# epfl-lts2/pygsp

Measured on AMD Instinct MI355X. Metric: filtered-vertices/sec (N·Nsig·K/s) + achieved HBM GB/s vs roofline, 1M-vertex K=30, higher is better.
Workload: dtype f64

## Files before the change

pygsp_amd/csrc/gspx_ctx.hip.h:

```cpp
#pragma once

struct Options {
  int64_t kernel = 0;
  int64_t vec = 0;
  int64_t rows_per_wave = 0;
  int64_t narrow_g_log2 = -1;
  int64_t waves_per_block = 4;
  int64_t calib_mix = 0;
  int64_t graph_launch = 2;
  int64_t tile_gather = 1;
  int64_t tile_workgroups = 0;
  int64_t knn_f32 = 1;
  int64_t tile_pad = 1;
  int64_t tile_min_row = 16;
  int64_t staged_copy = 1;
  int64_t staged_copy_min_mb = 32;
  int64_t copy_threads = 0;
  int64_t tile_regroup = 1;
  int64_t tile_acc_builds = 1;
  int64_t tile_lg = 0;
  int64_t edge_vertex_walk = 1;
  int64_t fuse_input = 1;
  int64_t tile_nt = -1;
  int64_t synthesis = 0;
  int64_t alternate_sweep = 1;
  int64_t xcd_remap = 1;
  int64_t combine = 0;
  int64_t ws_limit_mb = 65536;
  int64_t max_batch = 0;
  int64_t gather_rccl = 1;
  int64_t lds_pad_kb = 0;
  int64_t host_pipeline = 1;
  int64_t host_batch = 0;
  int64_t host_edge = 0;
  int64_t host_threads = 0;
  int64_t streamed_alloc = 1;
  int64_t layout_splits = 0;
};

struct gspx_ctx {
  int device = 0;
  int cu_count = 256;
  hipStream_t stream = nullptr;
  Options opt;
  DevMem ws_t;
  DevMem ws_r;
  DevMem ws_w;
  DevMem io_x, io_y;
  DevMem ws_spec;
  DevMem ws_sq, ws_sqp;
  HostPipe* pipe = nullptr;
  CopyStage* copy = nullptr;
  bool counted = false;
  std::mutex comms_mu;
  std::vector<struct gspx_comm*> comms;
  hipEvent_t ev[4] = {nullptr, nullptr, nullptr, nullptr};
  std::vector<hipEvent_t> ev_pool;
  double timing[5] = {0, 0, 0, 0, 0};
  int64_t step_kinds[2] = {0, 0};
  bool capturing = false;
  std::vector<unsigned char> seen_key;
  std::vector<unsigned char> graph_key;
  hipGraphExec_t graph_exec = nullptr;
  int64_t graph_kinds[2] = {0, 0};
};

static std::atomic<int> g_live_ctx[64];

static void replay_reset(gspx_ctx* ctx) {
  if (!ctx) return;
  ctx->seen_key.clear();
  ctx->graph_key.clear();
  if (ctx->graph_exec) {
    (void)hipGraphExecDestroy(ctx->graph_exec);
    ctx->graph_exec = nullptr;
  }
}

static int finish_timed(gspx_ctx* ctx, double* kernel_ms) {
  HIPCHK(hipGetLastError());
  HIPCHK(hipStreamSynchronize(ctx->stream));
  float f = 0;
  HIPCHK(hipEventElapsedTime(&f, ctx->ev[0], ctx->ev[1]));
  if (kernel_ms) *kernel_ms = f;
  return GSPX_OK;
}

struct gspx_buf {
  gspx_ctx* ctx = nullptr;
  DevMem mem;
  int64_t bytes = 0;
};

static std::atomic<uint64_t> g_generation{1};

struct gspx_graph {
  gspx_ctx* ctx = nullptr;
  const uint64_t generation = g_generation.fetch_add(1);
  int64_t N = 0;
  int dtype = GSPX_F64;
  bool from_w = false;
  int64_t nnz_l = 0;
// ... 93 lines not shown
    return set_err(GSPX_ERR_HIP, "hipStreamCreate failed: %s", hipGetErrorString(e));
  }
  for (int i = 0; i < 4; ++i) {
    e = hipEventCreate(&ctx->ev[i]);
    if (e != hipSuccess) {
      delete ctx;
      return set_err(GSPX_ERR_HIP, "hipEventCreate failed: %s", hipGetErrorString(e));
    }
  }
  *out = ctx;
  return GSPX_OK;
}

static void comm_invalidate_all(gspx_ctx* ctx);

extern "C" int gspx_ctx_destroy(gspx_ctx* ctx) {
  replay_reset(ctx);
  if (!ctx) return GSPX_OK;
  if (ctx->counted) g_live_ctx[ctx->device & 63].fetch_sub(1);
  comm_invalidate_all(ctx);
  if (ctx->graph_exec) {
    (void)hipGraphExecDestroy(ctx->graph_exec);
    ctx->graph_exec = nullptr;
  }
  (void)hipSetDevice(ctx->device);
  if (ctx->stream) (void)hipStreamSynchronize(ctx->stream);
  for (int i = 0; i < 4; ++i)
    if (ctx->ev[i]) (void)hipEventDestroy(ctx->ev[i]);
  for (hipEvent_t e : ctx->ev_pool) (void)hipEventDestroy(e);
  ctx->ws_t.release();
  ctx->ws_r.release();
  ctx->ws_w.release();
  ctx->io_x.release();
  ctx->io_y.release();
  ctx->ws_spec.release();
  ctx->ws_sq.release();
  ctx->ws_sqp.release();
  if (ctx->pipe) {
    ctx->pipe->destroy();
    delete ctx->pipe;
    ctx->pipe = nullptr;
  }
  if (ctx->copy) {
    ctx->copy->destroy();
    delete ctx->copy;
    ctx->copy = nullptr;
  }
  if (ctx->stream) (void)hipStreamDestroy(ctx->stream);
  delete ctx;
  return GSPX_OK;
}

extern "C" int gspx_ctx_sync(gspx_ctx* ctx) {
  if (!ctx) return set_err(GSPX_ERR_INVALID, "null ctx");
  HIPCHK(hipSetDevice(ctx->device));
  HIPCHK(hipStreamSynchronize(ctx->stream));
  return GSPX_OK;
}

struct OptionDef {
  const char* key;
  int64_t Options::*slot;
  bool (*ok)(int64_t);
  const char* refusal;
};
static const OptionDef OPTION_TABLE[] = {
    {"kernel", &Options::kernel, [](int64_t v) { return v == 0 || v == 1 || v == 2 || v == 5; },
     "kernel must be 0 (auto), 1 (panel), 2 (narrow) or 5 (LDS-staged)"},
    {"vec", &Options::vec, [](int64_t v) { return v == 0 || v == 1 || v == 2 || v == 4; }, "vec must be 0, 1, 2 or 4"},
    {"rows_per_wave", &Options::rows_per_wave, [](int64_t v) { return v >= 0 && v <= 1024; },
     "rows_per_wave must be in [0, 1024] (0 = auto)"},
    {"narrow_g_log2", &Options::narrow_g_log2, [](int64_t v) { return v >= -1 && v <= 6; },
     "narrow_g_log2 must be in [-1, 6] (-1 = auto)"},
    {"waves_per_block", &Options::waves_per_block, [](int64_t v) { return v == 4 || v == 8 || v == 16; },
     "waves_per_block must be 4, 8 or 16"},
    {"alternate_sweep", &Options::alternate_sweep, nullptr, nullptr},
    {"synthesis", &Options::synthesis, nullptr, nullptr},
    {"tile_gather", &Options::tile_gather, nullptr, nullptr},
    {"graph_launch", &Options::graph_launch, nullptr, nullptr},
    {"tile_workgroups", &Options::tile_workgroups, nullptr, nullptr},
    {"tile_lg", &Options::tile_lg, nullptr, nullptr},
    {"tile_regroup", &Options::tile_regroup, nullptr, nullptr},
    {"tile_acc_builds", &Options::tile_acc_builds, nullptr, nullptr},
    {"staged_copy", &Options::staged_copy, nullptr, nullptr},
    {"staged_copy_min_mb", &Options::staged_copy_min_mb, nullptr, nullptr},
    {"copy_threads", &Options::copy_threads, nullptr, nullptr},
    {"tile_min_row", &Options::tile_min_row, nullptr, nullptr},
    {"tile_pad", &Options::tile_pad, nullptr, nullptr},
    {"knn_f32", &Options::knn_f32, nullptr, nullptr},
    {"tile_nt", &Options::tile_nt, nullptr, nullptr},
    {"fuse_input", &Options::fuse_input, nullptr, nullptr},
    {"edge_vertex_walk", &Options::edge_vertex_walk, nullptr, nullptr},
    {"xcd_remap", &Options::xcd_remap, nullptr, nullptr},
    {"combine", &Options::combine, nullptr, nullptr},
    {"ws_limit_mb", &Options::ws_limit_mb, nullptr, nullptr},
    {"max_batch", &Options::max_batch, nullptr, nullptr},
    {"gather_rccl", &Options::gather_rccl, nullptr, nullptr},
    {"lds_pad_kb", &Options::lds_pad_kb, nullptr, nullptr},
    {"host_pipeline", &Options::host_pipeline, nullptr, nullptr},
    {"host_batch", &Options::host_batch, nullptr, nullptr},
    {"host_edge", &Options::host_edge, nullptr, nullptr},
    {"host_threads", &Options::host_threads, nullptr, nullptr},
    {"streamed_alloc", &Options::streamed_alloc, nullptr, nullptr},
    {"layout_splits", &Options::layout_splits, [](int64_t v) { return v >= 0 && v <= 65535; },
     "layout_splits must be in [0, 65535] (0 = automatic)"},
};

static const OptionDef* find_option(const char* key) {
  if (key)
    for (const OptionDef& d : OPTION_TABLE)
      if (!strcmp(key, d.key)) return &d;
  set_err(GSPX_ERR_INVALID, "unknown option '%s'", key ? key : "(null)");
  return nullptr;
}

extern "C" int gspx_ctx_set_option(gspx_ctx* ctx, const char* key, int64_t value) {
  replay_reset(ctx);
  if (!ctx) return set_err(GSPX_ERR_INVALID, "null ctx");
  const OptionDef* d = find_option(key);
  if (!d) return GSPX_ERR_INVALID;
  if (d->ok && !d->ok(value)) return set_err(GSPX_ERR_INVALID, "%s", d->refusal);
  ctx->opt.*d->slot = value;
  if (d->slot == &Options::streamed_alloc) {
    const bool on = value != 0;
    (void)hipSetDevice(ctx->device);
    for (DevMem* m : {&ctx->ws_t, &ctx->ws_r}) {
      if (!on && m->va_size) {
        (void)hipStreamSynchronize(ctx->stream);
        m->release();
      }
      m->streamed = on;
    }
  }
  return GSPX_OK;
}

extern "C" int gspx_ctx_get_option(gspx_ctx* ctx, const char* key, int64_t* value) {
  if (!ctx || !value) return set_err(GSPX_ERR_INVALID, "null argument");
  if (key && !strcmp(key, "retired_va_mb")) {
    *value = (int64_t)(g_retired_va_bytes.load() >> 20);
    return GSPX_OK;
  }
  const OptionDef* d = find_option(key);
  if (!d) return GSPX_ERR_INVALID;
  *value = ctx->opt.*d->slot;
  return GSPX_OK;
}

extern "C" int gspx_buf_alloc(gspx_ctx* ctx, int64_t bytes, gspx_buf** out) {
  if (!ctx || !out || bytes < 0) return set_err(GSPX_ERR_INVALID, "gspx_buf_alloc: bad argument");
  *out = nullptr;
  HIPCHK(hipSetDevice(ctx->device));
  gspx_buf* b = new gspx_buf();
  b->ctx = ctx;
  b->bytes = bytes;
  int rc = b->mem.alloc((size_t)bytes);
  if (rc != GSPX_OK) {
    delete b;
    return rc;
  }
  *out = b;
  return GSPX_OK;
}

extern "C" int gspx_buf_free(gspx_buf* b) {
  if (!b) return GSPX_OK;
// ... 170 lines not shown
```

pygsp_amd/csrc/gspx_poly.hip.h:

```cpp
#pragma once

struct PlanStep {
  double scale = 1.0, gamma = -1.0;
  int flush = 0;
  int final = 0;
  std::vector<double> w;
};

static void make_plan_fused(int nf, int M, const std::vector<double>& cp, bool acc_existing,
                            bool final_to_y, std::vector<PlanStep>& plan) {
  const int K = M - 1;
  plan.assign((size_t)K, PlanStep());
  int covered = -1;
  bool first = !acc_existing;
  for (int k = 1; k <= K; ++k) {
    PlanStep& st = plan[(size_t)k - 1];
    st.scale = (k == 1) ? 0.5 : 1.0;
    st.gamma = (k == 1) ? 0.0 : -1.0;
    st.w.assign((size_t)nf * 3, 0.0);
    const bool must = (k == K) || (k >= 2 && (k - 2) > covered);
    if (!must) continue;
    st.flush = first ? 1 : 2;
    first = false;
    st.final = (k == K && final_to_y) ? 1 : 0;
// ... 311 lines not shown
  if constexpr (sizeof(T) == 4) {
    if (vec == 2) kern = k_slot_dots<T, 2, 8>;
  }
  hipLaunchKernelGGL(kern, grid, dim3(256), 0, st, slots, S, slot_stride, (u32)pitch, N, (int)w, cwl, sd.part);
  const int64_t n = (int64_t)(2 * S - 1) * w;
  hipLaunchKernelGGL(k_dots_reduce, dim3((unsigned)((n + 63) / 64)), dim3(256), 0, st, sd.part, gx, n, (int)w, sd.out,
                     sd.ldo);
  return GSPX_OK;
}

struct CrossDots {
  const void* z;
  unsigned ldz;
  size_t zplane;
  int nf;
  double* out;
  size_t ldo;
  double* part;
};
static const int CROSS_PASS = 8, CROSS_FEW = 2;
static int cross_cs(int here, int vec) { return (here <= CROSS_FEW ? 16 : 8) / vec; }
template <typename T> static int cross_vec(unsigned w, unsigned pitch, const T* z, unsigned ldz) {
  return dots_vec<T>(w, pitch) == 2 && ldz % 2 == 0 && ((uintptr_t)z % (2 * sizeof(T))) == 0 ? 2 : 1;
}
static int cross_chunks(int M, int here, int vec) { return (M + cross_cs(here, vec) - 1) / cross_cs(here, vec); }
static int cross_gx(const gspx_ctx* ctx, int N, unsigned w, int M, int here, int vec) {
  const int cwl = sqnorm_cwl(w / vec);
  const int64_t rows = 4 * (int64_t)(64 >> cwl);
  const int64_t tiles = ((int64_t)N + rows - 1) / rows;
  const int64_t others = (((int64_t)(w / vec) + (1 << cwl) - 1) >> cwl) * cross_chunks(M, here, vec);
  const int64_t fit = ((int64_t)64 << 20) / ((int64_t)here * M * w * (int64_t)sizeof(double));
  const int64_t want = (8 * (int64_t)ctx->cu_count + others - 1) / others;
  return (int)std::max<int64_t>(1, std::min(std::min(tiles, want), fit));
}
static size_t cross_parts(const gspx_ctx* ctx, int N, unsigned w, int M, int nf) {
  size_t most = 0;
  for (int here : {std::min(nf, CROSS_PASS), nf % CROSS_PASS})
    for (int vec = 1; here > 0 && vec <= (w % 2 == 0 ? 2 : 1); ++vec)
      most = std::max(most, (size_t)cross_gx(ctx, N, w, M, here, vec) * (size_t)here * M * w);
  return most;
}

template <typename T>
static int launch_slot_cross_dots(gspx_ctx* ctx, const T* slots, int M, size_t slot_stride, unsigned pitch, int N,
                                  unsigned w, const int* perm, const CrossDots& cd, hipStream_t st) {
  const T* z = (const T*)cd.z;
  const int vec = cross_vec<T>(w, pitch, z, cd.ldz);
  const int cwl = sqnorm_cwl(w / vec);
  typedef void (*kern_t)(const T*, int, size_t, u32, const T*, int, size_t, u32, const int*, int, int, int, double*);
  for (int f0 = 0; f0 < cd.nf; f0 += CROSS_PASS) {
    const int here = std::min(CROSS_PASS, cd.nf - f0);
    const bool few = here <= CROSS_FEW;
    kern_t kern = few ? k_slot_cross_dots<T, 1, 16, CROSS_FEW> : k_slot_cross_dots<T, 1, 8, CROSS_PASS>;
    if constexpr (sizeof(T) == 4) {
      if (vec == 2) kern = few ? k_slot_cross_dots<T, 2, 8, CROSS_FEW> : k_slot_cross_dots<T, 2, 4, CROSS_PASS>;
    }
    const int gx = cross_gx(ctx, N, w, M, here, vec);
    const dim3 grid((unsigned)gx, (unsigned)cross_chunks(M, here, vec), (w / vec + (1u << cwl) - 1) >> cwl);
    hipLaunchKernelGGL(kern, grid, dim3(256), 0, st, slots, M, slot_stride, (u32)pitch, z + (size_t)f0 * cd.zplane, here,
                       cd.zplane, (u32)cd.ldz, perm, N, (int)w, cwl, cd.part);
    const int64_t n = (int64_t)here * M * w;
    hipLaunchKernelGGL(k_dots_reduce, dim3((unsigned)((n + 63) / 64)), dim3(256), 0, st, cd.part, gx, n, (int)w,
                       cd.out + (size_t)f0 * M * cd.ldo, cd.ldo);
  }
  return GSPX_OK;
}

struct SlotsUse {
  int (*fn)(gspx_ctx*, const void*, int, size_t, unsigned, int, unsigned, const int*, const void*, hipStream_t);
  const void* arg;
};

template <typename T> static bool tile_geometry(const gspx_graph* g, const Options& opt, unsigned ld) {
  constexpr int TVEC = 16 / (int)sizeof(T);
  const size_t U = (size_t)g->N * ld;
  return opt.tile_gather && g->gt_rows == GSPX_TILE_BR && (size_t)ld * sizeof(T) >= (size_t)opt.tile_min_row &&
         (ld % TVEC) == 0 && U * sizeof(T) < ((size_t)1 << 31) && (size_t)g->nnz_int * sizeof(T) < ((size_t)1 << 31);
}
template <typename T>
static bool tile_usable(const gspx_graph* g, const Options& opt, unsigned ld, const T* y, unsigned ldy) {
  constexpr int TVEC = 16 / (int)sizeof(T);
  return tile_geometry<T>(g, opt, ld) && (ldy % TVEC) == 0 && (((uintptr_t)y / sizeof(T)) % TVEC) == 0;
}
template <typename T>
static int launch_step_tile(gspx_graph* g, const Options& opt, TileArgs<T> t, unsigned ld, hipStream_t st,
                            const T* vals = nullptr) {
  const size_t rowb = (size_t)ld * sizeof(T);
  int lg = rowb <= 16 ? 1 : rowb <= 32 ? 2 : rowb <= 64 ? 4 : rowb <= 128 ? 8 : 16;
  if (opt.tile_lg == 8 || opt.tile_lg == 4 || opt.tile_lg == 2) lg = rowb <= 128 ? std::max(lg, (int)opt.tile_lg) : 16;
  const bool narrow = lg < 16;
  const int ncol = narrow ? 1 : (int)((rowb + 255) / 256);
  const int flavour = t.old_rows ? 1 : t.nin > 0 ? 2 : 0;
  typedef void (*kern_t)(const TileArgs<T>);
  static const kern_t wide[3][3] = {
      {k_step_tile<T, 0>, k_step_tile<T, 1>, k_step_tile<T, 2>},
      {k_step_tile<T, 0, 16, true>, k_step_tile<T, 1, 16, true>, k_step_tile<T, 2, 16, true>},
      {k_step_tile<T, 0, 16, false, true>, k_step_tile<T, 1, 16, false, true>, k_step_tile<T, 2, 16, false, true>}};
  static const kern_t slim[3][4] = {
      {k_step_tile<T, 1, 1, false, false, 64>, k_step_tile<T, 1, 2, false, false, 128>,
       k_step_tile<T, 1, 4, false, false, 256>, k_step_tile<T, 1, 8>},
      {k_step_tile<T, 1, 1, true, false, 64>, k_step_tile<T, 1, 2, true, false, 128>,
       k_step_tile<T, 1, 4, true, false, 256>, k_step_tile<T, 1, 8, true>},
      {k_step_tile<T, 1, 1, false, true, 64>, k_step_tile<T, 1, 2, false, true, 128>,
       k_step_tile<T, 1, 4, false, true, 256>, k_step_tile<T, 1, 8, false, true>}};
  kern_t kern = narrow ? slim[flavour][lg == 1 ? 0 : lg == 2 ? 1 : lg == 4 ? 2 : 3] : wide[flavour][ncol <= 2 ? ncol : 0];
  unsigned threads = narrow ? 64u * (unsigned)lg : 512u;
  const bool noacc = opt.tile_acc_builds && t.flush == 0 && !narrow && flavour == 0;
  if (noacc) {
    static const kern_t freek[3] = {k_step_tile<T, 0, 16, false, false, 512, 16, 0, false>,
                                    k_step_tile<T, 1, 16, false, false, 512, 16, 0, false>,
                                    k_step_tile<T, 2, 16, false, false, 512, 16, 0, false>};
    kern = freek[ncol <= 2 ? ncol : 0];
  }
  bool mix = false;
  if (opt.calib_mix && !narrow && flavour == 0) {
    static const kern_t mixk[2][3] = {
        {k_step_tile<T, 0, 16, false, false, 512, 16, 1>, k_step_tile<T, 1, 16, false, false, 512, 16, 1>,
         k_step_tile<T, 2, 16, false, false, 512, 16, 1>},
        {k_step_tile<T, 0, 16, false, false, 512, 16, 2>, k_step_tile<T, 1, 16, false, false, 512, 16, 2>,
         k_step_tile<T, 2, 16, false, false, 512, 16, 2>}};
    static const kern_t mixfree[2][3] = {
        {k_step_tile<T, 0, 16, false, false, 512, 16, 1, false>, k_step_tile<T, 1, 16, false, false, 512, 16, 1, false>,
         k_step_tile<T, 2, 16, false, false, 512, 16, 1, false>},
        {k_step_tile<T, 0, 16, false, false, 512, 16, 2, false>, k_step_tile<T, 1, 16, false, false, 512, 16, 2, false>,
         k_step_tile<T, 2, 16, false, false, 512, 16, 2, false>}};
    kern = (noacc ? mixfree : mixk)[opt.calib_mix == 2 ? 1 : 0][ncol <= 2 ? ncol : 0];
    mix = true;
  }
  const int pieces = (int)(rowb / 16);
  if (opt.tile_regroup && ncol == 1 && flavour != 1 && pieces < lg && !mix) {
#define GSPX_CL(LG_, CL_, NT_) \
  (flavour == 2 ? (kern_t)k_step_tile<T, 1, LG_, false, true, NT_, CL_> : (kern_t)k_step_tile<T, 1, LG_, false, false, NT_, CL_>)
    kern_t k2 = nullptr;
    unsigned nt2 = 0;
    if (lg == 4 && pieces == 3) k2 = GSPX_CL(4, 3, 192), nt2 = 192;
    else if (lg == 8 && pieces == 5) k2 = GSPX_CL(8, 5, 320), nt2 = 320;
    else if (lg == 16 && pieces == 10) k2 = GSPX_CL(16, 10, 320), nt2 = 320;
#undef GSPX_CL
    if (k2) kern = k2, threads = nt2;
  }
  size_t lds = g->gt_lds;
  if (lg < 8)
    lds = std::min(lds, (size_t)GSPX_TILE_MAXN1 * 16 * lg + (((size_t)g->gt_entmax * sizeof(T) + 15) & ~(size_t)15) +
                            (((size_t)g->gt_entmax + 15) & ~(size_t)15) + 64);
  if (lg < 8) lds = (lds + 2047) & ~(size_t)2047;
  int per_cu = 2;
  {
    struct Known { size_t attr = 0; std::map<size_t, int> fit; };
    static std::map<std::pair<const void*, int>, Known> known;
    static std::mutex lds_mu;
    std::lock_guard<std::mutex> lock(lds_mu);
    Known& k = known[std::make_pair((const void*)kern, g->ctx->device)];
    if (k.attr < lds) {
      HIPCHK(hipFuncSetAttribute((const void*)kern, hipFuncAttributeMaxDynamicSharedMemorySize, (int)lds));
      k.attr = lds;
    }
    if (lg < 8) {
      auto it = k.fit.find(lds);
      if (it == k.fit.end()) {
        int fit = 2;
        HIPCHK(hipOccupancyMaxActiveBlocksPerMultiprocessor(&fit, (const void*)kern, (int)threads, lds));
        it = k.fit.emplace(lds, std::max(2, std::min(fit, 16))).first;
      }
      per_cu = it->second;
    }
  }
  t.rowptr = g->rptr.as<int>();
  t.col = g->rcol.as<int>();
  t.val = vals ? vals : g->fval.as<T>();
  t.hdr = g->gt_hdr.as<int>();
  if (!t.s1rows) t.s1rows = g->gt_s1rows.as<int>();
  t.lidx = g->gt_lidx.as<unsigned char>();
  t.N = (int)g->N;
  t.ld = ld;
  t.panel_bytes = (unsigned)((size_t)g->N * ld * sizeof(T));
  t.val_bytes = (unsigned)((size_t)g->nnz_int * sizeof(T));
  t.lidx_bytes = (unsigned)((size_t)g->nnz_int);
  t.nb = g->gt_nb;
  t.ncol = ncol;
  t.per_xcd = (t.nb + 7) / 8;
  t.lds_bytes = (int)lds;
  unsigned nwg = (unsigned)std::max<int64_t>(8, ((int64_t)per_cu * g->ctx->cu_count) / 8 * 8);
  if (opt.tile_workgroups > 0)
    nwg = (unsigned)std::max<int64_t>(8, std::min<int64_t>(opt.tile_workgroups, 1 << 20) / 8 * 8);
  nwg = std::min(nwg, 8u * (unsigned)std::max(t.per_xcd, 1));
  t.nt = opt.tile_nt >= 0 ? (int)opt.tile_nt : ((size_t)g->N * ld * sizeof(T) >= ((size_t)192 << 20) ? 5 : 0);
  ++g->ctx->step_kinds[0];
  hipLaunchKernelGGL(kern, dim3(nwg), dim3(threads), lds, st, t);
  return GSPX_OK;
}

template <typename T>
static int prepare_coff(gspx_graph* g, const Shape& shape, unsigned ld, hipStream_t st) {
  if (shape.kernel == 5 && g->coff_ldb != ld * (unsigned)sizeof(T)) {
    CHK(g->coff.ensure(((size_t)g->nnz_int + 64) * sizeof(unsigned)));
    const int nb = std::max(1, (int)((g->N + 255) / 256));
    hipLaunchKernelGGL((k_coff<T>), dim3(nb), dim3(256), 0, st, g->rptr.as<int>(), g->rcol.as<int>(), (int)g->N,
                       ld * (unsigned)sizeof(T), g->coff.as<unsigned>());
    g->coff_ldb = ld * (unsigned)sizeof(T);
  }
  return GSPX_OK;
}

template <typename T> static int vec_cap(int v, unsigned ld, const T* p) {
  while (v > 1 && ((ld % v) != 0 || (((uintptr_t)p / sizeof(T)) % v) != 0)) v /= 2;
  return v;
}

struct WorkPanels {
  bool tile_direct, padded;
  unsigned ldw;
};
template <typename T>
static WorkPanels work_panels(const gspx_graph* g, const Options& opt, bool tiles, size_t planes, unsigned ld,
                              const T* y, unsigned ldy) {
  constexpr unsigned TVEC = 16 / (unsigned)sizeof(T);
  const unsigned ldp = (ld + TVEC - 1) / TVEC * TVEC;
  auto window = [&](unsigned w) { return planes * (size_t)g->N * w * sizeof(T) < ((size_t)1 << 31); };
  const bool pad_pays = opt.tile_pad == 2 || ld >= 2 ||
                        (size_t)g->nnz_int * (sizeof(T) + 4) >= ((size_t)20 << 20);
  WorkPanels p;
  p.tile_direct = tiles && tile_usable<T>(g, opt, ld, y, ldy) && window(ld);
// ... 7 lines not shown
  StepArgs<T> a{};
  a.rowptr = g->rptr.as<int>();
  a.col = g->rcol.as<int>();
  a.val = g->fval.as<T>();
  a.N = (int)g->N;
  a.ld = ld;
  a.curbytes = (u32)((size_t)g->N * ld * sizeof(T));
  a.y = y;
  a.ldy = ldy;
  a.perm = g->has_perm ? g->perm.as<int>() : nullptr;
  return a;
}

static int batch_events(gspx_ctx* ctx, size_t& ev_idx, hipEvent_t ev[4]) {
  for (int i = 0; i < 4; ++i) ev[i] = pool_event(ctx, ++ev_idx);
  if (!ev[0] || !ev[1] || !ev[2] || !ev[3]) return set_err(GSPX_ERR_HIP, "hipEventCreate failed");
  HIPCHK(hipEventRecord(ev[0], ctx->stream));
  return GSPX_OK;
}

static int batch_width(const gspx_graph* g, size_t elt, size_t panels, int64_t Nsig, int64_t* width) {
  const Options& opt = g->ctx->opt;
  const size_t rowb = (size_t)g->N * elt;
  int64_t max_ld = (int64_t)((((size_t)1 << 31) - 65536) / rowb);
  if (max_ld < 1)
    return set_err(GSPX_ERR_INVALID, "graph too large: one signal column exceeds 2 GiB");
  const size_t budget = (size_t)std::max<int64_t>(opt.ws_limit_mb, 1) << 20;
  max_ld = std::min<int64_t>(max_ld, std::max<int64_t>(1, (int64_t)(budget / (rowb * panels))));
  if (opt.max_batch > 0) max_ld = std::min<int64_t>(max_ld, opt.max_batch);
  if (max_ld < Nsig && max_ld >= 4) max_ld &= ~(int64_t)3;
  *width = max_ld;
  return GSPX_OK;
}

template <typename Batch>
static int run_batches(gspx_graph* g, int64_t Nsig, int64_t width, int steps, const Batch& batch) {
  gspx_ctx* ctx = g->ctx;
  size_t ev_idx = 0;
  HIPCHK(hipEventRecord(ctx->ev[0], ctx->stream));
  for (int64_t c0 = 0; c0 < Nsig; c0 += width)
    CHK(batch(c0, (unsigned)std::min<int64_t>(width, Nsig - c0), ev_idx));
  HIPCHK(hipEventRecord(ctx->ev[1], ctx->stream));
  HIPCHK(hipStreamSynchronize(ctx->stream));
  float ms = 0;
  HIPCHK(hipEventElapsedTime(&ms, ctx->ev[0], ctx->ev[1]));
  ctx->timing[0] = ms;
  double phase[3] = {0, 0, 0};
  for (size_t i = 0; i + 3 < ev_idx; i += 4)
    for (size_t j = 0; j < 3; ++j) {
      float t = 0;
      HIPCHK(hipEventElapsedTime(&t, ctx->ev_pool[i + j], ctx->ev_pool[i + j + 1]));
      phase[j] += t;
    }
  ctx->timing[1] = phase[1];
  ctx->timing[2] = (double)(ev_idx / 4) * steps;
  ctx->timing[3] = phase[0];
  ctx->timing[4] = phase[2];
  return GSPX_OK;
}

template <typename T>
static int run_batch(gspx_graph* g, int nf, int M, const std::vector<double>& cp, const T* x,
                     unsigned ldx, T* y, unsigned ldy, unsigned ld, bool deferred,
                     bool acc_existing, bool final_to_y, size_t& ev_idx, const SqNorms* sq = nullptr,
                     const SlotDots* sd = nullptr, const CrossDots* cd = nullptr, const SlotsUse* use = nullptr) {
  gspx_ctx* ctx = g->ctx;
  const Options& opt = ctx->opt;
  hipStream_t st = ctx->stream;
  const int N = (int)g->N;
  const int K = M - 1;
  const WorkPanels wp = work_panels<T>(g, opt, deferred || nf == 1, 1, ld, y, ldy);
  const bool tile_direct = wp.tile_direct, padded = wp.padded;
  const unsigned ldw = wp.ldw;
  const size_t U = (size_t)N * ldw;
  const Shape shape = choose_shape(opt, sizeof(T), ld, vec_cap(4, ldy, y));
  const int* perm = g->has_perm ? g->perm.as<int>() : nullptr;

  std::vector<PlanStep> plan;
  if (deferred)
    make_plan_deferred(nf, M, plan);
  else
    make_plan_fused(nf, M, cp, acc_existing, final_to_y, plan);

  std::vector<T> hw;
  if (deferred) {
    hw.resize((size_t)nf * M);
    for (size_t i = 0; i < hw.size(); ++i) hw[i] = (T)cp[i];
  } else {
    hw.resize((size_t)K * nf * 3);
    for (int k = 0; k < K; ++k)
      for (int j = 0; j < nf * 3; ++j) hw[(size_t)k * nf * 3 + j] = (T)plan[(size_t)k].w[(size_t)j];
  }
  const bool cap = ctx->capturing;
  if (!cap) {
    CHK(ctx->ws_w.ensure(hw.size() * sizeof(T) + 64));
    HIPCHK(hipMemcpyAsync(ctx->ws_w.p, hw.data(), hw.size() * sizeof(T), hipMemcpyHostToDevice, st));
    HIPCHK(hipStreamSynchronize(st));
  }

  const size_t nslots = deferred ? (size_t)M : 2;
  const size_t SU = U;
  CHK(ctx->ws_t.ensure(nslots * SU * sizeof(T) + 256));
  if (!deferred) CHK(ctx->ws_r.ensure((size_t)nf * U * sizeof(T) + 256));
  T* slots = ctx->ws_t.as<T>();
  T* racc = ctx->ws_r.as<T>();

  hipEvent_t ev[4] = {};
  if (!cap) CHK(batch_events(ctx, ev_idx, ev));
  const bool tile_ok = tile_direct || padded;
  const unsigned char* xb = (const unsigned char*)x;
  const unsigned char* yb = (const unsigned char*)y;
  const size_t xbytes = (size_t)N * ldx * sizeof(T), ybytes = (size_t)nf * N * ldy * sizeof(T);
  const bool fuse_in = tile_direct && !deferred && opt.fuse_input && g->gt_slow == 0 && ldx == ld &&
                       ((uintptr_t)x % 16) == 0 && (xb + xbytes <= yb || yb + ybytes <= xb) &&
                       (!g->has_perm || (g->gt_ns1 > 0 && (!cap || g->gt_s1nat.p)));
  if (fuse_in) {
    CHK(ensure_s1nat(g, st));
  } else if (padded) {
    const unsigned nb = (unsigned)std::min<size_t>((U + 255) / 256, 65536);
    hipLaunchKernelGGL((k_permute_in_pad<T>), dim3(nb), dim3(256), 0, st, x, ldx, slots, ldw, ld, N, perm);
  } else {
    launch_permute_in<T>(x, ldx, slots, ld, N, perm, vec_cap(shape.vec, ldx, x), st);
  }
  if (!cap) HIPCHK(hipEventRecord(ev[1], st));

  CHK(prepare_coff<T>(g, shape, ld, st));
  StepArgs<T> a = step_base<T>(g, ld, y, ldy);
  a.nf = nf;
  a.racc = racc;
  for (int k = 1; k <= K; ++k) {
    const PlanStep& ps = plan[(size_t)k - 1];
    if (tile_ok) {
      TileArgs<T> t{};
      if (deferred) {
        t.cur = slots + (size_t)(k - 1) * SU;
        t.old = (k >= 2 && ps.gamma != 0.0) ? slots + (size_t)(k - 2) * SU : t.cur;
        t.out = slots + (size_t)k * SU;
      } else {
        t.cur = slots + (size_t)((k - 1) & 1) * SU;
        t.old = ps.gamma == 0.0 ? t.cur : slots + (size_t)(k & 1) * SU;
        t.out = slots + (size_t)(k & 1) * SU;
        if (fuse_in && k == 1) {
          t.cur = x;
          t.old = x;
          t.s1rows = g->has_perm ? g->gt_s1nat.as<int>() : nullptr;
        } else if (fuse_in && k == 2) {
          t.old = x;
          t.old_rows = perm;
        }
      }
      t.racc = racc;
      t.y = y;
      t.ldy = ldy;
      t.perm = perm;
      t.scale = (T)ps.scale;
      t.gamma = (T)ps.gamma;
      t.beta = T(0);
      t.flush = ps.flush;
      t.final = padded ? 0 : ps.final;
      t.reverse = (opt.alternate_sweep && (k & 1)) ? 1 : 0;
      if (ps.flush) {
        t.wn = (T)ps.w[0];
        t.wc = (T)ps.w[1];
        t.wo = (T)ps.w[2];
      }
      CHK(launch_step_tile<T>(g, opt, t, ldw, st));
      continue;
    }
    if (deferred) {
      a.cur = slots + (size_t)(k - 1) * SU;
      a.old = k >= 2 ? slots + (size_t)(k - 2) * SU : slots;
      a.out = slots + (size_t)k * SU;
    } else {
      a.cur = slots + (size_t)((k - 1) & 1) * SU;
      a.old = slots + (size_t)(k & 1) * SU;
      a.out = slots + (size_t)(k & 1) * SU;
    }
    if (ps.gamma == 0.0) a.old = a.cur;
    a.scale = (T)ps.scale;
    a.gamma = (T)ps.gamma;
    a.flush = ps.flush;
    a.final = ps.final;
    a.reverse = (opt.alternate_sweep && (k & 1)) ? 1 : 0;
    a.wts = ctx->ws_w.as<T>() + (size_t)(k - 1) * nf * 3;
    launch_step<T>(ctx, a, shape, opt, st, g->coff.as<unsigned>());
  }
  if (!cap) HIPCHK(hipEventRecord(ev[2], st));
  if (deferred && sq) {
    CHK(launch_combine_sqnorm<T>(ctx, slots, M, SU, ldw, N, ld, *sq, st));
  } else if (deferred && sd) {
    CHK(launch_slot_dots<T>(ctx, slots, M, SU, ldw, N, ld, *sd, st));
  } else if (deferred && cd) {
    CHK(launch_slot_cross_dots<T>(ctx, slots, M, SU, ldw, N, ld, perm, *cd, st));
  } else if (deferred && use) {
    CHK(use->fn(ctx, slots, M, SU, ldw, N, ld, perm, use->arg, st));
  } else if (deferred) {
    launch_combine<T>(slots, M, SU, ctx->ws_w.as<T>(), M, nf, N, ld, y, ldy, (size_t)N * ldy, perm,
                      padded ? 1 : vec_cap(shape.vec, ldy, y), st, ldw);
  } else if (padded && final_to_y) {
    const unsigned nb = (unsigned)std::min<size_t>(((size_t)N * ld + 255) / 256, 65536);
    hipLaunchKernelGGL((k_permute_out_pad<T>), dim3(nb), dim3(256), 0, st, racc, ldw, y, ldy, ld, N, perm);
  }
  if (!cap) {
    HIPCHK(hipEventRecord(ev[3], st));
    HIPCHK(hipGetLastError());
  }
  return GSPX_OK;
}

template <typename T>
static int clenshaw_step(gspx_graph* g, const Options& opt, const WorkPanels& wp, const Shape& shape, StepArgs<T>& a,
                         int k, int K, const T* inp, const T* wts, int nin, const T* first, T* const B[2], T* y,
                         unsigned ldy, hipStream_t st) {
  gspx_ctx* ctx = g->ctx;
  const bool has_b2 = (k + 2 <= K);
  if (wp.tile_direct || wp.padded) {
    TileArgs<T> t{};
    t.cur = (k == K) ? first : B[(k + 1) & 1];
    t.old = (k < K && has_b2) ? B[k & 1] : t.cur;
    t.out = B[k & 1];
    t.racc = B[0];
    t.y = y;
    t.ldy = ldy;
    t.perm = a.perm;
    t.scale = (k == K) ? T(0) : (k == 0 ? T(0.5) : T(1));
    t.gamma = (k < K && has_b2) ? T(-1) : T(0);
    t.beta = T(0);
    t.inp = inp;
    t.wts = wts;
    t.nin = nin;
    t.flush = 0;
    t.final = (k == 0 && !wp.padded) ? 1 : 0;
    t.reverse = (opt.alternate_sweep && (k & 1)) ? 1 : 0;
    return launch_step_tile<T>(g, opt, t, wp.ldw, st);
  }
  a.nf = 1;
  a.nin = nin;
  a.racc = const_cast<T*>(inp);
  a.wts = wts;
  a.final = (k == 0) ? 1 : 0;
  a.flush = 0;
  if (k == K) {
    a.cur = first;
    a.old = first;
    a.out = B[k & 1];
    a.scale = T(0);
    a.gamma = T(0);
  } else {
    a.cur = B[(k + 1) & 1];
// ... 610 lines not shown
```

pygsp_amd/csrc/gspx_tile_kernels.hip.h:

```cpp
#pragma once

#include "gspx_kernels.hip.h"

namespace gspx {

template <typename T> struct TileArgs {
  const int* rowptr;
  const int* col;
  const T* val;
  const int* hdr;
  const int* s1rows;
  const u8* lidx;
  const T* cur;
  const T* old;
  const int* old_rows;
  T* out;
  T* racc;
  T* y;
  const int* perm;
  int N;
  u32 ld, ldy;
  u32 panel_bytes, val_bytes, lidx_bytes;
  int nb, ncol, per_xcd;
  int lds_bytes;
  T scale, gamma;
  T beta;
  T wn, wc, wo;
  const T* inp;
  const T* wts;
  int nin;
  int flush;
  int final;
  int reverse;
  int nt;
};

constexpr int GSPX_TILE_BR = 64;
constexpr int GSPX_TILE_MAXN1 = 160;

template <typename T, int NCOL, int LG, bool OLDNAT, bool ACC = true> struct TileSchedule {
  static constexpr bool PF = !OLDNAT;
  static constexpr bool TILE_LAST = PF && LG == 16;
  static constexpr bool PF_ENTRIES = PF;
  static constexpr bool META_AFTER = !OLDNAT && LG == 16 && NCOL == 0;
  static constexpr bool EARLY_OLD = !ACC && PF && LG == 16 && NCOL == 2 && sizeof(T) == 4;
};

template <typename T, int NCOL, int LG = 16, bool OLDNAT = false, bool INS = false, int NT = 512, int CL = LG,
          int MIX = 0, bool ACC = true>
__global__ __launch_bounds__(NT, 4) void k_step_tile(const TileArgs<T> a) {
  static_assert(NT == 512 || (NT == 64 * LG && NCOL == 1) || (CL < LG && NCOL == 1 && NT % 64 == 0 && NT % CL == 0),
                "narrow builds: one row per group, one chunk per row");
  constexpr int BR = GSPX_TILE_BR;
  static_assert(CL <= LG && (BR % (NT / CL)) == 0, "compute groups must tile the block's rows");
  constexpr int MAXN1 = GSPX_TILE_MAXN1;
  typedef TileSchedule<T, NCOL, LG, OLDNAT, ACC> Sched;
  constexpr bool PF = Sched::PF;
  constexpr bool META_AFTER = Sched::META_AFTER;
  constexpr bool TILE_LAST = Sched::TILE_LAST;
  constexpr bool PF_ENTRIES = Sched::PF_ENTRIES;
  constexpr bool EARLY_OLD = Sched::EARLY_OLD;
  static_assert(ACC || (!OLDNAT && !INS && CL == LG), "flush-free builds: the plain flavour only");
  constexpr int VEC = 16 / (int)sizeof(T);
  typedef typename VT<T, VEC>::t V;
  typedef __attribute__((address_space(3))) void* lds_ptr;
  extern __shared__ __attribute__((aligned(16))) unsigned char gspx_smem[];

  const int tid = threadIdx.x;
  constexpr int NGD = NT / LG;
  constexpr int NG = NT / CL;
  constexpr int NE = (512 + NT - 1) / NT;
  constexpr int RPG = BR / NG;
  constexpr int ST = (MAXN1 + NGD - 1) / NGD;
  constexpr int RB = LG * 16;
  const int lane_d = tid & (LG - 1);
  const int grp_d = tid / LG;
  const int lane16 = CL == LG ? lane_d : tid % CL;
  const int grp = CL == LG ? grp_d : tid / CL;
  const int wave = tid >> 6;
  const int nwx = (int)(gridDim.x >> 3);
  const int xlo = (int)(blockIdx.x & 7) * a.per_xcd;
  int k1 = xlo + a.per_xcd;
  if (k1 > a.nb) k1 = a.nb;
  const int k0 = xlo + (int)(blockIdx.x >> 3);
  if (k0 >= k1) return;

  constexpr u32 POISON = 0x80000000u;
  const rsrc_t rcur = __builtin_amdgcn_make_buffer_rsrc((void*)a.cur, 0, a.panel_bytes, 0x00020000);
  const rsrc_t rold = __builtin_amdgcn_make_buffer_rsrc((void*)a.old, 0, a.panel_bytes, 0x00020000);
  const rsrc_t rra = __builtin_amdgcn_make_buffer_rsrc((void*)a.racc, 0, a.panel_bytes, 0x00020000);
  const rsrc_t rv = __builtin_amdgcn_make_buffer_rsrc((void*)a.val, 0, a.val_bytes, 0x00020000);
  const rsrc_t ri = __builtin_amdgcn_make_buffer_rsrc((void*)a.lidx, 0, a.lidx_bytes, 0x00020000);
  const u32 ldb = a.ld * (u32)sizeof(T);

  struct Meta { int rows[ST]; int rp[RPG + 1]; int orow[OLDNAT ? RPG : 1]; };
  const int xflip = xlo + k1 - 1;
  const bool rev = a.reverse != 0;
  auto phys = [&](int p) { return rev ? xflip - p : p; };
  auto load_hdr = [&](int p) { return *(const int4*)(a.hdr + (size_t)phys(p) * 4); };
  auto uniform = [](int4 h) {
    int4 u;
    u.x = __builtin_amdgcn_readfirstlane(h.x); u.y = __builtin_amdgcn_readfirstlane(h.y);
    u.z = __builtin_amdgcn_readfirstlane(h.z); u.w = __builtin_amdgcn_readfirstlane(h.w);
    return u;
  };
  auto load_meta = [&](int k, const int4& h) {
    Meta m;
    const int n1 = h.y;
#pragma unroll
    for (int t = 0; t < ST; ++t) {
      const int u = grp_d + NGD * t;
      m.rows[t] = a.s1rows[h.x + (u < n1 ? u : 0)];
    }
    int r = phys(k) * BR + grp * RPG;
#pragma unroll
    for (int t = 0; t < RPG + 1; ++t) m.rp[t] = a.rowptr[(r + t) <= a.N ? (r + t) : a.N];
    if constexpr (OLDNAT) {
#pragma unroll
      for (int t = 0; t < RPG; ++t) m.orow[t] = a.old_rows[(r + t) < a.N ? (r + t) : a.N - 1];
    }
    return m;
  };
  V* const tile = (V*)gspx_smem;
  auto stage = [&](const Meta& m, int n1, u32 cb) {
#pragma unroll
    for (int t = 0; t < ST; ++t) {
      if (grp_d + NGD * t < n1)
        __builtin_amdgcn_raw_ptr_buffer_load_lds(rcur, (lds_ptr)(gspx_smem + (wave * (64 / LG) + NGD * t) * RB), 16,
                                                 (u32)m.rows[t] * ldb + cb, 0, 0, 0);
    }
  };
  auto chunk_off_d = [&](int c) {
    const u32 col0 = (c * LG + lane_d) * VEC;
    return col0 < a.ld ? col0 * (u32)sizeof(T) : POISON;
  };
  auto chunk_off = [&](int c) {
    const u32 col0 = (c * LG + lane16) * VEC;
    return col0 < a.ld ? col0 * (u32)sizeof(T) : POISON;
  };

  V ov[RPG], ra[ACC ? RPG : 1];
  V ov2[EARLY_OLD ? RPG : 1];
  u32x4 ev[NE], ei = 0;
#pragma unroll
  for (int q = 0; q < NE; ++q) ev[q] = 0;
  auto prefetch_rows = [&](const Meta& m, int blk, int c, V (&dst)[RPG]) {
    const int r0 = phys(blk) * BR + grp * RPG;
    const u32 cb = chunk_off(c);
#pragma unroll
    for (int t = 0; t < RPG; ++t) {
      const u32 off = (r0 + t < a.N && cb != POISON) ? (u32)(r0 + t) * ldb + cb : POISON;
      u32 oo = a.gamma != T(0) ? off : POISON;
      if constexpr (OLDNAT) oo = (off != POISON && a.gamma != T(0)) ? (u32)m.orow[t] * ldb + cb : POISON;
      if (a.nt & 4) dst[t] = __builtin_bit_cast(V, __builtin_amdgcn_raw_buffer_load_b128(rold, oo, 0, 2));
      else dst[t] = VT<T, VEC>::bload(rold, oo);
      if constexpr (ACC) {
        const u32 ro = a.flush == 2 ? off : POISON;
        if (a.nt & 2) ra[t] = __builtin_bit_cast(V, __builtin_amdgcn_raw_buffer_load_b128(rra, ro, 0, 2));
        else ra[t] = VT<T, VEC>::bload(rra, ro);
      }
    }
  };
  auto prefetch_entries = [&](const int4& h) {
    const int nv16 = (h.w * (int)sizeof(T) + 15) >> 4, ni16 = (h.w + 15) >> 4;
    const u32 io = tid < ni16 ? (u32)h.z + tid * 16u : POISON;
#pragma unroll
    for (int q = 0; q < NE; ++q) {
      const int i = tid + q * NT;
      const u32 vo = i < nv16 ? (u32)h.z * (u32)sizeof(T) + i * 16u : POISON;
      if (a.nt & 1) ev[q] = __builtin_amdgcn_raw_buffer_load_b128(rv, vo, 0, 2);
      else ev[q] = __builtin_amdgcn_raw_buffer_load_b128(rv, vo, 0, 0);
    }
    if (a.nt & 1) ei = __builtin_amdgcn_raw_buffer_load_b128(ri, io, 0, 2);
    else ei = __builtin_amdgcn_raw_buffer_load_b128(ri, io, 0, 0);
  };

  int4 H = uniform(load_hdr(k0));
  Meta M = load_meta(k0, H);
  int k = k0, kn = k0 + nwx, knn = k0 + 2 * nwx;
  int4 Hn = uniform(load_hdr(kn < k1 ? kn : k0));
  if constexpr (!TILE_LAST) {
    if (H.y >= 0) stage(M, H.y, chunk_off_d(0));
  }
  if constexpr (EARLY_OLD) {
#pragma unroll
    for (int t = 0; t < RPG; ++t) ov[t] = 0, ov2[t] = 0;
    if (a.gamma != T(0)) prefetch_rows(M, k0, 0, ov);
  } else if constexpr (PF) {
    prefetch_rows(M, k0, 0, ov);
  }
  if constexpr (PF_ENTRIES) {
    if (H.y >= 0) prefetch_entries(H);
  }
  if constexpr (TILE_LAST) {
    __builtin_amdgcn_sched_barrier(0);
    if (H.y >= 0) stage(M, H.y, chunk_off_d(0));
    __builtin_amdgcn_sched_barrier(0);
  }

  auto pass = [&](const int c, const bool first, const bool last, V (&ovc)[RPG], V (&ovn)[RPG])
                  __attribute__((always_inline)) {
    const int n1 = H.y, rp0 = H.z, ent = H.w;
    const bool fast = n1 >= 0;
    T* const mval = (T*)(tile + (fast ? n1 : 0) * LG);
    u8* const midx = (u8*)(mval + ent);
    const int row0 = phys(k) * BR + grp * RPG;
    int rs[RPG + 1];
#pragma unroll
    for (int t = 0; t < RPG + 1; ++t) rs[t] = M.rp[t] & ~3;
    const u32 col0 = (c * LG + lane16) * VEC;
    const bool on = col0 < a.ld;
    const u32 cb = on ? col0 * (u32)sizeof(T) : POISON;
    if constexpr (!PF) prefetch_rows(M, k, c, ovc);
    V ins[INS ? RPG : 1];
#pragma unroll
    for (int t = 0; t < (INS ? RPG : 1); ++t) ins[t] = 0;
    if constexpr (INS) {
      const rsrc_t rin = __builtin_amdgcn_make_buffer_rsrc((void*)a.inp, 0, a.panel_bytes * (u32)a.nin, 0x00020000);
      for (int f = 0; f < a.nin; ++f) {
        const T w = a.wts[f];
#pragma unroll
        for (int t = 0; t < RPG; ++t) {
          const u32 off = (row0 + t < a.N) ? (u32)(row0 + t) * ldb + cb : POISON;
          ins[t] += w * VT<T, VEC>::bload(rin, off == POISON ? POISON : off + (u32)f * a.panel_bytes);
        }
      }
    }
    if constexpr (!PF_ENTRIES) {
      if (first && fast) prefetch_entries(H);
    }
    int4 Hv = Hn;
    if constexpr (!META_AFTER) {
      if (last) {
        M = load_meta(kn < k1 ? kn : k, Hn);
        Hv = load_hdr(knn < k1 ? knn : k);
      }
    }
    __builtin_amdgcn_sched_barrier(0);
    if (first && fast) {
      const int nv16 = (ent * (int)sizeof(T) + 15) >> 4, ni16 = (ent + 15) >> 4;
#pragma unroll
      for (int q = 0; q < NE; ++q)
        if (tid + q * NT < nv16) *(u32x4*)((unsigned char*)mval + (tid + q * NT) * 16) = ev[q];
      if (tid < ni16) *(u32x4*)((unsigned char*)midx + tid * 16) = ei;
      for (int i = tid + NE * NT; i < nv16; i += NT)
        *(u32x4*)((unsigned char*)mval + i * 16) =
            __builtin_amdgcn_raw_buffer_load_b128(rv, (u32)rp0 * (u32)sizeof(T) + i * 16u, 0, 0);
      for (int i = tid + NT; i < ni16; i += NT)
        *(u32x4*)((unsigned char*)midx + i * 16) =
            __builtin_amdgcn_raw_buffer_load_b128(ri, (u32)rp0 + i * 16u, 0, 0);
    }
    if constexpr (TILE_LAST && !META_AFTER) {
      constexpr int NMETA = ST + RPG + 1 + 1;
      static_assert(NMETA < 16, "vmcnt immediate");
      if (last && !INS) __builtin_amdgcn_s_waitcnt(0x0070 | NMETA);
      else __builtin_amdgcn_s_waitcnt(0x0070);
    } else {
      __builtin_amdgcn_s_waitcnt(0x0070);
    }
    if constexpr (MIX != 2) __syncthreads();
    if constexpr (META_AFTER) {
      if (last) {
        M = load_meta(kn < k1 ? kn : k, Hn);
        Hv = load_hdr(knn < k1 ? knn : k);
      }
    }
    if constexpr (EARLY_OLD) {
      if ((!last || kn < k1) && a.gamma != T(0)) prefetch_rows(M, last ? kn : k, last ? 0 : c + 1, ovn);
    }
    __builtin_amdgcn_sched_barrier(0);
    V nv[RPG], res[ACC ? RPG : 1];
#pragma unroll
    for (int t = 0; t < RPG; ++t) {
      const int s = rs[t], e = rs[t + 1];
      V acc = 0, self = 0;
      if (MIX && fast) {
        self = tile[(int)midx[s - rp0] * LG + lane16];
        acc = mval[s - rp0] * self;
      } else if (fast) {
        acc = lds_row_dot<T, V, LG, u8>(mval + (s - rp0), midx + (s - rp0), row0 + t < a.N ? e - s : 0, tile, lane16,
                                        self);
      } else if (row0 + t < a.N) {
        for (int j = s; j < e; ++j) {
          const int cc = a.col[j];
          const V xv = VT<T, VEC>::bload(rcur, cc < a.N ? (u32)cc * ldb + cb : POISON);
          if (j == s) self = xv;
          acc += a.val[j] * xv;
        }
      }
      if constexpr (ACC) {
        nv[t] = a.scale * acc + a.gamma * ovc[t] + a.beta * self;
      } else {
        nv[t] = __builtin_elementwise_fma((V)a.beta, self, __builtin_elementwise_fma((V)a.gamma, ovc[t], a.scale * acc));
      }
      if constexpr (INS) nv[t] += ins[t];
      if constexpr (ACC) {
        res[t] = a.wn * nv[t] + a.wc * self + a.wo * ovc[t];
        if (a.flush == 2) res[t] += ra[t];
      }
    }
    __builtin_amdgcn_s_waitcnt(0xC07F);
    if constexpr (MIX != 2) __builtin_amdgcn_s_barrier();
    bool more = true;
    if (last) {
      const int4 Hnn = uniform(Hv);
      H = Hn;
      Hn = Hnn;
      more = kn < k1;
    }
    __builtin_amdgcn_sched_barrier(0);
    if constexpr (!PF) {
      if (more && H.y >= 0) stage(M, H.y, chunk_off_d(last ? 0 : c + 1));
    }
#pragma unroll
    for (int t = 0; t < RPG; ++t) {
      const int row = row0 + t;
      if (row < a.N && on) {
        if (a.final && (!ACC || !a.flush)) {
          const size_t orow = a.perm ? (size_t)a.perm[row] : (size_t)row;
          *(V*)(a.y + orow * a.ldy + col0) = nv[t];
          continue;
        }
        if (a.nt & 8) __builtin_nontemporal_store(nv[t], (V*)(a.out + (size_t)row * a.ld + col0));
        else *(V*)(a.out + (size_t)row * a.ld + col0) = nv[t];
        if constexpr (ACC) {
          if (a.flush) {
            if (a.final) {
              const size_t orow = a.perm ? (size_t)a.perm[row] : (size_t)row;
              *(V*)(a.y + orow * a.ldy + col0) = res[t];
            } else {
              if (a.nt & 2) __builtin_nontemporal_store(res[t], (V*)(a.racc + (size_t)row * a.ld + col0));
              else *(V*)(a.racc + (size_t)row * a.ld + col0) = res[t];
            }
          }
        }
      }
    }
    __builtin_amdgcn_sched_barrier(0);
    if constexpr (PF) {
      if (more) {
        const int nc = last ? 0 : c + 1;
        if constexpr (!TILE_LAST) {
          if (H.y >= 0) stage(M, H.y, chunk_off_d(nc));
        }
        if constexpr (!EARLY_OLD) prefetch_rows(M, last ? kn : k, nc, ovn);
        if constexpr (PF_ENTRIES) {
          if (last && H.y >= 0) prefetch_entries(H);
        }
        if constexpr (TILE_LAST) {
          __builtin_amdgcn_sched_barrier(0);
          if (H.y >= 0) stage(M, H.y, chunk_off_d(nc));
          __builtin_amdgcn_sched_barrier(0);
        }
      }
    }
    if (last) {
      k = kn;
      kn = knn;
      knn += nwx;
    }
    return more;
  };
  if constexpr (EARLY_OLD) {
    static_assert(NCOL == 2, "an even number of passes per block");
    for (;;) {
      pass(0, true, false, ov, ov2);
      if (!pass(1, false, true, ov2, ov)) break;
    }
  } else {
    for (;;) {
      if constexpr (NCOL == 1) {
        if (!pass(0, true, true, ov, ov)) break;
      } else if constexpr (NCOL == 2) {
        pass(0, true, false, ov, ov);
        if (!pass(1, false, true, ov, ov)) break;
      } else {
        bool more = true;
        for (int c = 0; c < a.ncol; ++c) more = pass(c, c == 0, c == a.ncol - 1, ov, ov);
        if (!more) break;
      }
    }
  }
}

}

namespace gspx {

constexpr int GSPX_TILE_SORTCAP = 4096;
constexpr int GSPX_TILE_TMPCAP = 256;

__global__ __launch_bounds__(256) void k_tiles_unique(const int* __restrict__ rowptr,
                                                      const int* __restrict__ col, int N, int nb,
                                                      int* __restrict__ tmp, int* __restrict__ n1) {
  constexpr int BR = GSPX_TILE_BR;
  __shared__ unsigned keys[GSPX_TILE_SORTCAP];
  __shared__ int wsum[4];
  const int b = blockIdx.x;
  const int r0 = b * BR, r1 = min(r0 + BR, N);
  const int e0 = rowptr[r0] & ~3, e1 = rowptr[r1] & ~3;
// ... 101 lines not shown
```

Measured before the change: 191.7 billion.

## Add specialized tile kernels for first and last Chebyshev steps, skip redundant traffic

Adds edge-step specializations of the tiled step kernel. The last flushing step no longer writes the recurrence vector it will never read. The first flush (step 2 on the caller's panel) skips reading the accumulator and uses the prefetch schedule. The host-side weight upload and stream sync are also skipped when the tile path takes weights directly, and the accumulation is rewritten as FMAs. This trims HBM traffic and a host sync at the cost of more kernel instantiations and divergent code paths.

```diff
diff --git a/pygsp_amd/csrc/gspx_ctx.hip.h b/pygsp_amd/csrc/gspx_ctx.hip.h
--- a/pygsp_amd/csrc/gspx_ctx.hip.h
+++ b/pygsp_amd/csrc/gspx_ctx.hip.h
@@ -18,6 +18,7 @@
   int64_t copy_threads = 0;
   int64_t tile_regroup = 1;
   int64_t tile_acc_builds = 1;
+  int64_t tile_edge_builds = 1;
   int64_t tile_lg = 0;
   int64_t edge_vertex_walk = 1;
   int64_t fuse_input = 1;
@@ -277,6 +278,8 @@
     {"tile_lg", &Options::tile_lg, nullptr, nullptr},
     {"tile_regroup", &Options::tile_regroup, nullptr, nullptr},
     {"tile_acc_builds", &Options::tile_acc_builds, nullptr, nullptr},
+    {"tile_edge_builds", &Options::tile_edge_builds, [](int64_t v) { return v >= 0 && v <= 15; },
+     "tile_edge_builds must be 0, 1 or a sum of 2, 4 and 8"},
     {"staged_copy", &Options::staged_copy, nullptr, nullptr},
     {"staged_copy_min_mb", &Options::staged_copy_min_mb, nullptr, nullptr},
     {"copy_threads", &Options::copy_threads, nullptr, nullptr},
diff --git a/pygsp_amd/csrc/gspx_poly.hip.h b/pygsp_amd/csrc/gspx_poly.hip.h
--- a/pygsp_amd/csrc/gspx_poly.hip.h
+++ b/pygsp_amd/csrc/gspx_poly.hip.h
@@ -417,9 +417,14 @@
   constexpr int TVEC = 16 / (int)sizeof(T);
   return tile_geometry<T>(g, opt, ld) && (ldy % TVEC) == 0 && (((uintptr_t)y / sizeof(T)) % TVEC) == 0;
 }
+static const int EDGE_ITEM_NOSTORE = 2, EDGE_ITEM_FIRST = 4, EDGE_ITEM_UPLOAD = 8;
+static int edge_items(const Options& opt) {
+  const int all = EDGE_ITEM_NOSTORE | EDGE_ITEM_FIRST | EDGE_ITEM_UPLOAD;
+  return opt.tile_edge_builds == 1 ? all : (int)(opt.tile_edge_builds & all);
+}
 template <typename T>
 static int launch_step_tile(gspx_graph* g, const Options& opt, TileArgs<T> t, unsigned ld, hipStream_t st,
-                            const T* vals = nullptr) {
+                            const T* vals = nullptr, int edge = 0) {
   const size_t rowb = (size_t)ld * sizeof(T);
   int lg = rowb <= 16 ? 1 : rowb <= 32 ? 2 : rowb <= 64 ? 4 : rowb <= 128 ? 8 : 16;
   if (opt.tile_lg == 8 || opt.tile_lg == 4 || opt.tile_lg == 2) lg = rowb <= 128 ? std::max(lg, (int)opt.tile_lg) : 16;
@@ -472,7 +477,20 @@
     else if (lg == 8 && pieces == 5) k2 = GSPX_CL(8, 5, 320), nt2 = 320;
     else if (lg == 16 && pieces == 10) k2 = GSPX_CL(16, 10, 320), nt2 = 320;
 #undef GSPX_CL
-    if (k2) kern = k2, threads = nt2;
+    if (k2) kern = k2, threads = nt2, edge = 0;
+  }
+  if (edge && !narrow && !mix && flavour != 2) {
+#define GSPX_EDGE(NC_, ON_, E_) k_step_tile<T, NC_, 16, ON_, false, 512, 16, 0, true, E_>
+    static const kern_t lastk[2][3] = {
+        {GSPX_EDGE(0, false, EDGE_NOSTORE), GSPX_EDGE(1, false, EDGE_NOSTORE), GSPX_EDGE(2, false, EDGE_NOSTORE)},
+        {nullptr, GSPX_EDGE(1, true, EDGE_NOSTORE), GSPX_EDGE(2, true, EDGE_NOSTORE)}};
+    const int nc = ncol <= 2 ? ncol : 0;
+    if (edge == EDGE_NOSTORE && t.flush != 0) {
+      if (lastk[flavour][nc]) kern = lastk[flavour][nc];
+    } else if (edge == EDGE_FIRST && flavour == 1 && nc == 0 && t.flush == 1 && !t.final) {
+      kern = GSPX_EDGE(0, true, EDGE_FIRST);
+    }
+#undef GSPX_EDGE
   }
   size_t lds = g->gt_lds;
   if (lg < 8)
@@ -646,17 +664,19 @@
   else
     make_plan_fused(nf, M, cp, acc_existing, final_to_y, plan);
 
-  std::vector<T> hw;
-  if (deferred) {
-    hw.resize((size_t)nf * M);
-    for (size_t i = 0; i < hw.size(); ++i) hw[i] = (T)cp[i];
-  } else {
-    hw.resize((size_t)K * nf * 3);
-    for (int k = 0; k < K; ++k)
-      for (int j = 0; j < nf * 3; ++j) hw[(size_t)k * nf * 3 + j] = (T)plan[(size_t)k].w[(size_t)j];
-  }
+  const int edges = edge_items(opt);
   const bool cap = ctx->capturing;
-  if (!cap) {
+  const bool weights_read = deferred || !(wp.tile_direct || wp.padded) || !(edges & EDGE_ITEM_UPLOAD);
+  if (!cap && weights_read) {
+    std::vector<T> hw;
+    if (deferred) {
+      hw.resize((size_t)nf * M);
+      for (size_t i = 0; i < hw.size(); ++i) hw[i] = (T)cp[i];
+    } else {
+      hw.resize((size_t)K * nf * 3);
+      for (int k = 0; k < K; ++k)
+        for (int j = 0; j < nf * 3; ++j) hw[(size_t)k * nf * 3 + j] = (T)plan[(size_t)k].w[(size_t)j];
+    }
     CHK(ctx->ws_w.ensure(hw.size() * sizeof(T) + 64));
     HIPCHK(hipMemcpyAsync(ctx->ws_w.p, hw.data(), hw.size() * sizeof(T), hipMemcpyHostToDevice, st));
     HIPCHK(hipStreamSynchronize(st));
@@ -728,7 +748,12 @@
         t.wc = (T)ps.w[1];
         t.wo = (T)ps.w[2];
       }
-      CHK(launch_step_tile<T>(g, opt, t, ldw, st));
+      int edge = 0;
+      if (!deferred && k == K && ps.flush && (edges & EDGE_ITEM_NOSTORE))
+        edge = EDGE_NOSTORE;
+      else if (!deferred && k == 2 && t.old_rows && ps.flush == 1 && (edges & EDGE_ITEM_FIRST))
+        edge = EDGE_FIRST;
+      CHK(launch_step_tile<T>(g, opt, t, ldw, st, nullptr, edge));
       continue;
     }
     if (deferred) {
diff --git a/pygsp_amd/csrc/gspx_tile_kernels.hip.h b/pygsp_amd/csrc/gspx_tile_kernels.hip.h
--- a/pygsp_amd/csrc/gspx_tile_kernels.hip.h
+++ b/pygsp_amd/csrc/gspx_tile_kernels.hip.h
@@ -38,23 +38,30 @@
 constexpr int GSPX_TILE_BR = 64;
 constexpr int GSPX_TILE_MAXN1 = 160;
 
-template <typename T, int NCOL, int LG, bool OLDNAT, bool ACC = true> struct TileSchedule {
-  static constexpr bool PF = !OLDNAT;
+constexpr int EDGE_NOSTORE = 1, EDGE_FIRST = 2;
+template <typename T, int NCOL, int LG, bool OLDNAT, bool ACC = true, int EDGE = 0> struct TileSchedule {
+  static constexpr bool PF = !OLDNAT || (EDGE & EDGE_FIRST) != 0;
   static constexpr bool TILE_LAST = PF && LG == 16;
   static constexpr bool PF_ENTRIES = PF;
-  static constexpr bool META_AFTER = !OLDNAT && LG == 16 && NCOL == 0;
+  static constexpr bool META_AFTER = PF && LG == 16 && NCOL == 0;
   static constexpr bool EARLY_OLD = !ACC && PF && LG == 16 && NCOL == 2 && sizeof(T) == 4;
 };
 
 template <typename T, int NCOL, int LG = 16, bool OLDNAT = false, bool INS = false, int NT = 512, int CL = LG,
-          int MIX = 0, bool ACC = true>
+          int MIX = 0, bool ACC = true, int EDGE = 0>
 __global__ __launch_bounds__(NT, 4) void k_step_tile(const TileArgs<T> a) {
+  static_assert(EDGE == 0 || (ACC && !INS && !MIX && LG == 16 && CL == LG && NT == 512),
+                "edge builds: the wide plain and OLDNAT flavours only");
+  static_assert(!(EDGE & EDGE_FIRST) || (OLDNAT && NCOL == 0 && EDGE == EDGE_FIRST),
+                "first flush: step 2 on the caller's panel, rows of several chunks");
+  constexpr bool NOSTORE = (EDGE & EDGE_NOSTORE) != 0, FIRST = (EDGE & EDGE_FIRST) != 0;
+  constexpr bool RA = ACC && !FIRST;
   static_assert(NT == 512 || (NT == 64 * LG && NCOL == 1) || (CL < LG && NCOL == 1 && NT % 64 == 0 && NT % CL == 0),
                 "narrow builds: one row per group, one chunk per row");
   constexpr int BR = GSPX_TILE_BR;
   static_assert(CL <= LG && (BR % (NT / CL)) == 0, "compute groups must tile the block's rows");
   constexpr int MAXN1 = GSPX_TILE_MAXN1;
-  typedef TileSchedule<T, NCOL, LG, OLDNAT, ACC> Sched;
+  typedef TileSchedule<T, NCOL, LG, OLDNAT, ACC, EDGE> Sched;
   constexpr bool PF = Sched::PF;
   constexpr bool META_AFTER = Sched::META_AFTER;
   constexpr bool TILE_LAST = Sched::TILE_LAST;
@@ -139,7 +146,7 @@
     return col0 < a.ld ? col0 * (u32)sizeof(T) : POISON;
   };
 
-  V ov[RPG], ra[ACC ? RPG : 1];
+  V ov[RPG], ra[RA ? RPG : 1];
   V ov2[EARLY_OLD ? RPG : 1];
   u32x4 ev[NE], ei = 0;
 #pragma unroll
@@ -154,7 +161,7 @@
       if constexpr (OLDNAT) oo = (off != POISON && a.gamma != T(0)) ? (u32)m.orow[t] * ldb + cb : POISON;
       if (a.nt & 4) dst[t] = __builtin_bit_cast(V, __builtin_amdgcn_raw_buffer_load_b128(rold, oo, 0, 2));
       else dst[t] = VT<T, VEC>::bload(rold, oo);
-      if constexpr (ACC) {
+      if constexpr (RA) {
         const u32 ro = a.flush == 2 ? off : POISON;
         if (a.nt & 2) ra[t] = __builtin_bit_cast(V, __builtin_amdgcn_raw_buffer_load_b128(rra, ro, 0, 2));
         else ra[t] = VT<T, VEC>::bload(rra, ro);
@@ -288,15 +295,20 @@
           acc += a.val[j] * xv;
         }
       }
-      if constexpr (ACC) {
+      if constexpr (ACC && !EDGE) {
         nv[t] = a.scale * acc + a.gamma * ovc[t] + a.beta * self;
       } else {
         nv[t] = __builtin_elementwise_fma((V)a.beta, self, __builtin_elementwise_fma((V)a.gamma, ovc[t], a.scale * acc));
       }
       if constexpr (INS) nv[t] += ins[t];
-      if constexpr (ACC) {
+      if constexpr (ACC && !EDGE) {
         res[t] = a.wn * nv[t] + a.wc * self + a.wo * ovc[t];
         if (a.flush == 2) res[t] += ra[t];
+      } else if constexpr (ACC) {
+        res[t] = __builtin_elementwise_fma((V)a.wo, ovc[t], __builtin_elementwise_fma((V)a.wc, self, a.wn * nv[t]));
+        if constexpr (RA) {
+          if (a.flush == 2) res[t] += ra[t];
+        }
       }
     }
     __builtin_amdgcn_s_waitcnt(0xC07F);
@@ -316,6 +328,23 @@
     for (int t = 0; t < RPG; ++t) {
       const int row = row0 + t;
       if (row < a.N && on) {
+        if constexpr (NOSTORE) {
+          if (a.final) {
+            const size_t orow = a.perm ? (size_t)a.perm[row] : (size_t)row;
+            *(V*)(a.y + orow * a.ldy + col0) = res[t];
+          } else {
+            if (a.nt & 2) __builtin_nontemporal_store(res[t], (V*)(a.racc + (size_t)row * a.ld + col0));
+            else *(V*)(a.racc + (size_t)row * a.ld + col0) = res[t];
+          }
+          continue;
+        }
+        if constexpr (FIRST) {
+          if (a.nt & 8) __builtin_nontemporal_store(nv[t], (V*)(a.out + (size_t)row * a.ld + col0));
+          else *(V*)(a.out + (size_t)row * a.ld + col0) = nv[t];
+          if (a.nt & 2) __builtin_nontemporal_store(res[t], (V*)(a.racc + (size_t)row * a.ld + col0));
+          else *(V*)(a.racc + (size_t)row * a.ld + col0) = res[t];
+          continue;
+        }
         if (a.final && (!ACC || !a.flush)) {
           const size_t orow = a.perm ? (size_t)a.perm[row] : (size_t)row;
           *(V*)(a.y + orow * a.ldy + col0) = nv[t];
```

Result: no change. 193.5 billion (median of 6 runs) (+0.9%).
